# koide3/small_gicp

Hardware: AMD Instinct MI355X
Metric: GICP iterations/sec (1M<->1M pts) (higher is better)
Workload: dtype f32; 1 GPU; C3: GICP, per-point covariances k=20, 1000000 target <-> 1000000 source points, max_corr_dist 1.0 m; parallelism=single GPU

## Files before the change

### include/small_gicp_amd_debug.h

```cpp
#ifndef SMALL_GICP_AMD_DEBUG_H
#define SMALL_GICP_AMD_DEBUG_H

#include "small_gicp_amd.h"

#ifdef __cplusplus
extern "C" {
#endif

int sga_problem_set_search_stats(sga_context* ctx, sga_problem* pb, int enabled);
int sga_problem_get_search_stats(sga_context* ctx, const sga_problem* pb, int* leaves_per_point);
int sga_problem_get_sorted_points(sga_context* ctx, const sga_problem* pb, float* xyzw);
int sga_problem_get_last_plan(const sga_problem* pb, int out[8]);
int sga_problem_get_grid_stats(const sga_problem* pb, uint64_t out[6]);
void sga_set_grid_mode(int mode, long long min_points);
void sga_set_knn_wave_max(long long max_points);
int sga_index_spacing(const sga_index* index, double* spacing);
int sga_debug_kd_tree(sga_context* ctx, const sga_index* index, int* depth, float* nodes, float* xyzw);
int sga_debug_index_bbox(const sga_index* index, float lo[3], float hi[3]);
int sga_debug_forest_launches(unsigned long long* launches);
int sga_debug_voxelgrid_plan(const sga_cloud* cloud, double leaf, int out[9]);
int sga_debug_voxelgrid_batch_plan(const sga_cloud* const* clouds, size_t count, double leaf, int out[6]);
int sga_debug_voxelgrid_batch_launches(unsigned long long* launches);
int sga_debug_set_voxelgrid_epoch(sga_context* ctx, unsigned epoch);
int sga_debug_timer_start(sga_context* ctx);
int sga_debug_timer_stop(sga_context* ctx, double* ms);
#define SGA_FRAME_CHECK_DOUBLES 32
void sga_debug_shard_frame_pack(const double origin[3], double out[SGA_FRAME_CHECK_DOUBLES]);
// ... 11 lines not shown
```

### small_gicp_amd/_lib.py

```python
import ctypes as C
import os
import sys

_HERE = os.path.dirname(os.path.abspath(__file__))
LIB_PATH = os.environ.get("SGA_LIB_PATH") or os.path.join(_HERE, "lib", "libsmall_gicp_amd.so")

SGA_OK = 0
ICP, PLANE_ICP, GICP = 0, 1, 2
FLAT_NORMALS, FLAT_COVS = 1, 2
ROBUST_NONE, ROBUST_HUBER, ROBUST_CAUCHY = 0, 1, 2
LEVENBERG_MARQUARDT, GAUSS_NEWTON = 0, 1
MATH_FP32, MATH_FP64 = 0, 1
ACCUM_DOUBLES = 30


class SgaError(RuntimeError):
    pass


class FactorParams(C.Structure):
    _fields_ = [("factor_kind", C.c_int), ("robust_kind", C.c_int), ("robust_c", C.c_double), ("max_dist_sq", C.c_double), ("math_mode", C.c_int)]


class RegistrationSettingC(C.Structure):
# ... 112 lines not shown
    ("sga_linearize_per_point", C.c_int, [_vp, _vp, C.POINTER(FactorParams), _dp, _dp, C.POINTER(C.c_ubyte)]),
    ("sga_problem_get_factors", C.c_int, [_vp, _vp, C.POINTER(C.c_int64), _fp]),
    ("sga_context_set_stream_ordered", C.c_int, [_vp, C.c_int]),
    ("sga_context_set_profiling", C.c_int, [_vp, C.c_int]),
    ("sga_context_get_kernel_ms", C.c_int, [_vp, _dp, C.POINTER(C.c_uint64), _dp, C.POINTER(C.c_uint64)]),
    ("sga_context_get_comm_ms", C.c_int, [_vp, _dp, C.POINTER(C.c_uint64)]),
    ("sga_context_get_search_ms", C.c_int, [_vp, _dp, C.POINTER(C.c_uint64)]),
    ("sga_context_get_pass_ms", C.c_int, [_vp, _dp, C.POINTER(C.c_uint64), _dp, C.POINTER(C.c_uint64), _dp]),
    ("sga_set_warm_limit", None, [C.c_double]),
    ("sga_set_error_model", None, [C.c_int]),
    ("sga_problem_set_search_stats", C.c_int, [C.c_void_p, C.c_void_p, C.c_int]),
    ("sga_problem_get_search_stats", C.c_int, [C.c_void_p, C.c_void_p, C.c_void_p]),
    ("sga_problem_get_sorted_points", C.c_int, [C.c_void_p, C.c_void_p, C.c_void_p]),
    ("sga_problem_get_grid_stats", C.c_int, [C.c_void_p, C.POINTER(C.c_uint64)]),
    ("sga_problem_get_last_plan", C.c_int, [C.c_void_p, C.POINTER(C.c_int)]),
    ("sga_set_grid_mode", None, [C.c_int, C.c_longlong]),
    ("sga_host_alloc", C.c_int, [C.c_size_t, C.POINTER(C.c_void_p)]),
    ("sga_host_free", C.c_int, [C.c_void_p]),
    ("sga_index_spacing", C.c_int, [C.c_void_p, C.POINTER(C.c_double)]),
    ("sga_set_knn_wave_max", None, [C.c_longlong]),
    ("sga_debug_kd_tree", C.c_int, [C.c_void_p, C.c_void_p, C.POINTER(C.c_int), C.c_void_p, C.c_void_p]),
    ("sga_debug_voxelgrid_plan", C.c_int, [C.c_void_p, C.c_double, C.POINTER(C.c_int)]),
    ("sga_debug_set_voxelgrid_epoch", C.c_int, [C.c_void_p, C.c_uint]),
    ("sga_debug_timer_start", C.c_int, [C.c_void_p]),
    ("sga_debug_timer_stop", C.c_int, [C.c_void_p, C.POINTER(C.c_double)]),
    ("sga_debug_shard_frame_pack", None, [C.POINTER(C.c_double), C.POINTER(C.c_double)]),
    ("sga_debug_shard_frame_agree", C.c_int, [C.POINTER(C.c_double)]),
    ("sga_debug_reduce_rows", C.c_int, [C.c_void_p, C.c_void_p, C.c_int, C.c_int, C.c_void_p]),
    ("sga_debug_reduce_stamps", C.c_int, [C.c_void_p]),
    ("sga_debug_kd_trips", C.c_int, [C.c_void_p]),
# ... 60 lines not shown
```

### small_gicp_amd/api.py

```python
import ctypes as C

import numpy as np

from . import _lib
from ._lib import GICP, ICP, PLANE_ICP, FactorParams, RegistrationSettingC, ResultC, check, load

_FACTOR_BY_NAME = {"ICP": ICP, "PLANE_ICP": PLANE_ICP, "GICP": GICP, "VGICP": GICP}


def _fp(a):
    return None if a is None else a.ctypes.data_as(C.POINTER(C.c_float))


def _dp(a):
    return None if a is None else a.ctypes.data_as(C.POINTER(C.c_double))


def _T16(T):
    T = np.eye(4) if T is None else np.asarray(T, dtype=np.float64).reshape(4, 4)
    return np.ascontiguousarray(T.T).reshape(16)


class Context:

# ... 740 lines not shown
    def factors(self):
        n = self.source.size()
        ti = np.empty(n, np.int64)
        m6 = np.empty((n, 6), np.float32)
        check(load().sga_problem_get_factors(self.ctx.h, self.h, ti.ctypes.data_as(C.POINTER(C.c_int64)), _fp(m6)))
        return ti, m6

    ROUTES = ("factors", "grid", "certify", "fused_lane", "fused_queue", "queue", "lane")

    def last_plan(self):
        out = (C.c_int * 8)()
        check(load().sga_problem_get_last_plan(self.h, out))
        v = list(out)
        return {"route": self.ROUTES[v[0]], "warm": bool(v[1]), "grid": bool(v[2]), "pts": v[3], "tail": bool(v[4]), "chunk_tiles": v[5], "reduce_rows": v[6], "reduce_groups": v[7]}

    def align(self, setting, init_T=None):
        res = ResultC()
        t16 = _T16(init_T)
        check(load().sga_align_problem(self.ctx.h, self.h, _dp(t16), C.byref(setting), C.byref(res)))
        return RegistrationResult(res)

    def search_stats(self, enable=None):
        if enable is not None:
            check(load().sga_problem_set_search_stats(self.ctx.h, self.h, 1 if enable else 0))
            return None
        out = np.zeros(len(self.source), dtype=np.int32)
        check(load().sga_problem_get_search_stats(self.ctx.h, self.h, out.ctypes.data_as(C.c_void_p)))
        return out

    def sorted_points(self):
# ... 387 lines not shown
```

### small_gicp_amd/csrc/common.hpp

```cpp
#pragma once
#include <hip/hip_runtime.h>

#include <atomic>
#include <cstdarg>
#include <cstdint>
#include <cstdio>
#include <cstdlib>
#include <cstring>
#include <string>
#include <vector>

#include "../../include/small_gicp_amd.h"
#include "../../include/small_gicp_amd_debug.h"

namespace sga {

void set_error(const char* fmt, ...);
int fail(int code, const char* fmt, ...);

#define SGA_HIP(expr)                                                                                             \
  do {                                                                                                            \
    hipError_t _e = (expr);                                                                                       \
    if (_e != hipSuccess) return ::sga::fail(SGA_ERR_HIP, "%s:%d %s -> %s", __FILE__, __LINE__, #expr, hipGetErrorString(_e)); \
  } while (0)
// ... 218 lines not shown
  double src_origin[3] = {0, 0, 0};
  bool frame_checked = false;
  bool has_normals = false, has_covs = false;
  sga::DevBuf<float4> pts;
  sga::DevBuf<sga::Cov8> cov;
  const float4* pts_view = nullptr;
  const sga::Cov8* cov_view = nullptr;
  const float4* src_pts() const { return pts_view ? pts_view : pts.p; }
  const sga::Cov8* src_cov() const { return cov_view ? cov_view : cov.p; }
  sga::DevBuf<int> corr;
  sga::DevBuf<int> hint;
  sga::DevBuf<int> hint2;
  sga::DevBuf<float> rex;
  sga::DevBuf<int> dbg_leaves;
  sga::DevBuf<uint32_t> walked;
  bool state_fresh = false;
  double T_prev[16] = {0};
  bool prev_valid = false;
  int prev_math = 0;
  int lin_factor = -1;
  double lin_T[16] = {0};
  bool maha_valid = false;
  int last_math = 0;
  float bbox_lo[3] = {0, 0, 0}, bbox_hi[3] = {0, 0, 0};
  uint64_t cold_passes = 0, warm_passes = 0;
  uint64_t grid_passes = 0;
  sga::DevBuf<uint32_t> grid_stats;
  bool grid_stats_pending = false;
  uint64_t grid_open_total = 0, grid_ring_total = 0;
  double grid_open_frac = 0.0;
  sga::DevBuf<uint32_t> tile_cost, tile_order;
// ... 15 lines not shown
```

### small_gicp_amd/csrc/linearize.hip

```cpp
#include <algorithm>
#include <type_traits>

#include "batch.hpp"
#include "common.hpp"
#include "device_math.hpp"
#include "uniform.hpp"
#include "cell_grid.hpp"
#include "kd_search.hpp"
#include "projective.hpp"
#include "voxel_hash.hpp"
#include "notes.hpp"
#include "pass_layout.hpp"
#include "search_stage.hpp"
#include "factor_stage.hpp"
#include "reduce_rows.hpp"

void sga_profile_collect_pending(sga_context* ctx);

namespace sga {

int comm_allreduce_sum(sga_context* ctx, double* d_buf, size_t count);
template <typename Real>
int grid_search_pass(sga_context* ctx, const sga_index* idx, const float4* src_pts, int n, const Rigid<Real>& T, float reach2, int* nn, int* nn2, float* rex, uint32_t* stats);
int grid_rings_for(const sga_index* idx, double reach);
// ... 54 lines not shown
  uint32_t node = 1;
  int depth = 0, sp = 0;
  KdState s = kd_state(p.bound2, 0.f);

  for (;;) {
    while (tile < tile_end && q_count <= kQueueCap - 64) {
      const int i = tile * 64 + lane;
      bool need = i < p.n;
      float fx = 0.f, fy = 0.f, fz = 0.f, slack = 0.f;
      int seed = -1, cand2 = -1;
      if (need) {
        const float4 ps = p.src_pts[i];
        Real x, y, z;
        transform_point<Real>(p.T, ps.x, ps.y, ps.z, x, y, z);
        fx = static_cast<float>(x), fy = static_cast<float>(y), fz = static_cast<float>(z);
        seed = p.nn[i];
        cand2 = p.nn2[i];
        if constexpr (CHECK) {
          Real ox, oy, oz;
          transform_point<Real>(p.T_prev, ps.x, ps.y, ps.z, ox, oy, oz);
          const float moved = sqrtf(kd_dist2(static_cast<float>(ox), static_cast<float>(oy), static_cast<float>(oz), fx, fy, fz));
          float d1 = INFINITY, d2 = INFINITY;
          if (seed >= 0) {
            const float4 c = p.kd.pts[seed];
            d1 = kd_dist2(c.x, c.y, c.z, fx, fy, fz);
          }
          if (cand2 >= 0) {
            const float4 c = p.kd.pts[cand2];
            d2 = kd_dist2(c.x, c.y, c.z, fx, fy, fz);
          }
          const bool swap = cand2 >= 0 && (d2 < d1 || (d2 == d1 && cand2 < seed));
          const int best = swap ? cand2 : seed;
// ... 479 lines not shown
    acc += wave_sum_f64(static_cast<double>(e));
  }
  if (lane == 0) sh_e[wave] = acc;
  __syncthreads();
  if (threadIdx.x == 0) {
    double s = 0.0;
    for (int w = 0; w < kTile / 64; w++) s += sh_e[w];
    if (p.tail.enabled)
      __hip_atomic_store(&p.partials[blockIdx.x], s, __ATOMIC_RELAXED, __HIP_MEMORY_SCOPE_AGENT);
    else
      p.partials[blockIdx.x] = s;
  }
  if (p.tail.enabled) fused_tail(p.tail, p.partials, gridDim.x, 1, 1);
}

__global__ __launch_bounds__(1024) void tile_order_kernel(const uint32_t* __restrict__ cost, uint32_t* __restrict__ order, int num_tiles) {
  __shared__ uint32_t hist[64], start[64];
  const int per_xcd = num_tiles >> 3;
  const int x = blockIdx.x, first = x * per_xcd;
  if (threadIdx.x < 64) hist[threadIdx.x] = 0u;
  __syncthreads();
  for (int k = threadIdx.x; k < per_xcd; k += blockDim.x) atomicAdd(&hist[63u - min(63u, cost[first + k] >> 8)], 1u);
  __syncthreads();
  if (threadIdx.x == 0) {
    uint32_t acc = 0u;
    for (int b = 0; b < 64; b++) {
      start[b] = acc;
      acc += hist[b];
    }
  }
  __syncthreads();
  for (int k = threadIdx.x; k < per_xcd; k += blockDim.x) {
    const uint32_t pos = atomicAdd(&start[63u - min(63u, cost[first + k] >> 8)], 1u);
    order[first + pos] = static_cast<uint32_t>(first + k);
  }
  if (x == 0)
    for (int t = 8 * per_xcd + threadIdx.x; t < num_tiles; t += blockDim.x) order[t] = static_cast<uint32_t>(t);
}

template <typename T>
static T env_or(const char* name, T d) {
  const char* s = getenv(name);
  return s == nullptr ? d : std::is_floating_point_v<T> ? static_cast<T>(atof(s)) : static_cast<T>(atoll(s));
}

constexpr int kLinPts = 4;
constexpr int kLinPtsMin = 750000;
constexpr int kLinPtsMinF64 = 131072;

static double g_warm_delta = env_or("SGA_WARM_DELTA", 0.1);

static int g_search_queue = env_or("SGA_SEARCH_QUEUE", 2);
constexpr double kQueueDelta = 0.02;
static int g_chunk_tiles_cold = env_or("SGA_CHUNK_COLD", 4);
// ... 222 lines not shown

  const int math = sizeof(Real) == 4 ? SGA_MATH_FP32 : SGA_MATH_FP64;
  const double displacement = (!voxel && p.n > 0 && pb->prev_valid && pb->prev_math == math) ? max_displacement(T, pb->T_prev, pb->bbox_lo, pb->bbox_hi) : INFINITY;
  const double unit = voxel ? 1.0 : routing_unit(idx);
  NNParams<Real> q{};
  q.src_pts = pb->src_pts();
  q.n = p.n;
  q.kd = p.kd;
  q.T = p.T;
  q.within2 = p.bound2;
  q.slack_min = static_cast<float>(kSlackMin * unit), q.slack_max = static_cast<float>(kSlackMax * unit);
  q.cert_pad = std::max(g_cert_pad, 0.f);
  q.bound2 = p.bound2 * (1.f + kSearchMargin) * (1.f + kSearchMargin);
  q.nn = pb->hint.p, q.nn2 = pb->hint2.p, q.rex = pb->rex.p, q.walked = pb->walked.p;
  q.fast = g_fast_scan;
  q.leaves = pb->dbg_leaves.n >= pb->n ? pb->dbg_leaves.p : nullptr;

  const PassPlan plan = plan_pass<Real>(ctx, pb, q, displacement, unit, host_rejector);
  p.num_tiles = factor_tiles(p.n, plan.pts);
  const int blocks = grid_blocks(p.num_tiles);
  p.tail = FusedTail{plan.tail ? 1 : 0, ctx->d_ticket.p, d_out30, out_n, host, seq};
  q.check = plan.warm ? 1 : 0;
  if (plan.warm) q.T_prev = rigid_from_colmajor<Real>(pb->T_prev);
  if (plan.grid) {
    q.grid_walk = g_grid_walk;
    q.grid = make_grid_view(idx);
  }
  q.chunk_tiles = plan.chunk_tiles;

  const bool timed = ctx->profiling && (ctx->lin_seq++ % ctx->profile_period) == 0;
  if (timed) {
    sga_profile_collect_pending(ctx);
    (void)hipEventRecord(ctx->ev0, ctx->stream);
    ctx->pending_warm = plan.warm;
  }
  int rows = p.n > 0 ? blocks : 0;
  const bool first_pass = !pb->prev_valid;
  if (!voxel) pb->prev_valid = false;
  pb->state_fresh = false;
  if (plan.route != Route::kFactors) {
    if (q.leaves != nullptr) SGA_HIP(hipMemsetAsync(q.leaves, 0, pb->n * sizeof(int), ctx->stream));
    if (plan.grid && (first_pass || (plan.route != Route::kGrid && !plan.warm))) pb->grid_open_frac = 0.0;
    pb->order_tiles = 0;
    const size_t words = static_cast<size_t>(p.kd.depth);
    const dim3 sgrid((p.n + kSearchBlock - 1) / kSearchBlock), sblock(kSearchBlock);
    switch (plan.route) {
      case Route::kGrid:
        if (pb->grid_stats.n < 4) {
          SGA_TRY(pb->grid_stats.alloc(4));
          SGA_HIP(hipMemsetAsync(pb->grid_stats.p, 0, 4 * sizeof(uint32_t), ctx->stream));
        }
        SGA_TRY(grid_search_pass<Real>(ctx, idx, pb->src_pts(), p.n, p.T, q.bound2, pb->hint.p, pb->hint2.p, pb->rex.p, pb->grid_stats.p));
        pb->grid_passes++;
        break;
// ... 79 lines not shown
    }
  }
  if (p.n > 0 && !plan.fused()) {
    with_factor(fp->factor_kind, [&](auto f) {
      constexpr int F = decltype(f)::value;
      if (flat)
        launch_linearize<Real, F, 2>(ctx->stream, p, blocks, plan.pts);
      else if (proj) {
        hipLaunchKernelGGL((projective_linearize_kernel<Real, F, 1>), dim3(blocks), dim3(kTile), 0, ctx->stream, p, make_proj_view(idx));
      } else if (voxel) {
        if constexpr (F != SGA_PLANE_ICP) launch_linearize<Real, F, 1>(ctx->stream, p, blocks, plan.pts);
      } else
        launch_linearize<Real, F, 0>(ctx->stream, p, blocks, plan.pts);
    });
  }
  if (!plan.tail) launch_reduce(ctx, pb->partials.p, rows, ncols, kRow, pb->partials.p + partial_rows(pb->n) * kRow, d_out30, out_n, host, seq, true, plan.route == Route::kGrid ? pb->grid_stats.p : nullptr);
  pb->grid_stats_pending = plan.route == Route::kGrid && !plan.tail && out_n > kStatsCol + 1;
  {
    const int lp[8] = {static_cast<int>(plan.route), plan.warm, plan.grid, plan.pts, plan.tail, plan.chunk_tiles, plan.tail ? 0 : rows, plan.tail ? 0 : reduce_groups(rows)};
    std::copy(lp, lp + 8, pb->last_plan);
  }
  if (timed) {
    (void)hipEventRecord(ctx->ev1, ctx->stream);
    ctx->pending |= 1;
  }
  if (plan.order_record) {
    hipLaunchKernelGGL(tile_order_kernel, dim3(8), dim3(1024), 0, ctx->stream, pb->tile_cost.p, pb->tile_order.p, rows);
    pb->order_tiles = static_cast<unsigned>(rows);
    pb->order_stream = ctx->stream;
  }
  SGA_HIP(hipGetLastError());
  pb->last_math = math;
  pb->lin_factor = fp->factor_kind;
  memcpy(pb->lin_T, T, sizeof(pb->lin_T));
  pb->maha_valid = p.store_maha != 0;
  if (!voxel) {
    memcpy(pb->T_prev, T, sizeof(pb->T_prev));
    pb->prev_valid = true;
    pb->prev_math = math;
    if (plan.warm)
      pb->warm_passes++;
    else
// ... 331 lines not shown
    d.pair = k;
    prefix[a] = blocks;
    blocks += (d.ntiles + 7) / 8 * 8;
    pairs[a] = d;
  }
  prefix[order.size()] = blocks;
  const int nactive = static_cast<int>(order.size());
  const unsigned long long seq = ++bt->seq;
  SGA_HIP(hipMemcpyAsync(bt->d_round.p, bt->h_round, batch_round_bytes(count), hipMemcpyHostToDevice, ctx->stream));
  const int* d_prefix = reinterpret_cast<const int*>(bt->d_round.p);
  const BatchPair* d_pairs = reinterpret_cast<const BatchPair*>(bt->d_round.p + batch_pairs_offset(count));
  for (int k : order) {
    sga_problem* pb = bt->problems[k];
    pb->prev_valid = false;
    pb->model_valid = false;
    pb->state_fresh = false;
    pb->order_tiles = 0;
    if (bt->tiles[k] == 0 && pb->n > 0) SGA_HIP(hipMemsetAsync(pb->corr.p, 0xff, pb->n * sizeof(int), ctx->stream));
  }
  if (blocks > 0) {
    const size_t lds = static_cast<size_t>(std::max(bt->max_depth, 3)) * 64 * sizeof(uint32_t);
    with_factor(fp->factor_kind, [&](auto f) { hipLaunchKernelGGL((batch_search_linearize_kernel<decltype(f)::value>), dim3(blocks), dim3(64), lds, ctx->stream, d_prefix, d_pairs, nactive); });
  }
  hipLaunchKernelGGL(batch_reduce_rows_kernel, dim3(nactive), dim3(kReduceSlices * kCols), 0, ctx->stream, d_pairs, bt->ticket.p, bt->h_out_dev, bt->h_out_dev + count * kRow, seq);
  SGA_HIP(hipGetLastError());
  int rc = wait_result(ctx, seq, bt->h_out + count * kRow);
  if (rc != SGA_OK) {
    (void)hipMemsetAsync(bt->ticket.p, 0, sizeof(unsigned), ctx->stream);
    return rc;
  }
  for (size_t a = 0; a < order.size(); a++) {
// ... 84 lines not shown
  if (enabled) return pb->dbg_leaves.alloc(pb->n);
  pb->dbg_leaves.release();
  return SGA_OK;
}
int sga_problem_get_sorted_points(sga_context* ctx, const sga_problem* pb, float* xyzw) {
  if (!ctx || !pb || !xyzw) return fail(SGA_ERR_INVALID, "null argument");
  if (pb->n == 0) return SGA_OK;
  SGA_ENTER(ctx);
  SGA_HIP(hipMemcpyAsync(xyzw, pb->src_pts(), pb->n * sizeof(float4), hipMemcpyDeviceToHost, ctx->stream));
  SGA_HIP(hipStreamSynchronize(ctx->stream));
  return SGA_OK;
}
int sga_problem_get_last_plan(const sga_problem* pb, int out[8]) {
  if (!pb || !out) return fail(SGA_ERR_INVALID, "null argument");
  std::copy(pb->last_plan, pb->last_plan + 8, out);
  return SGA_OK;
}
int sga_problem_get_search_stats(sga_context* ctx, const sga_problem* pb, int* leaves_per_point) {
  if (!ctx || !pb || !leaves_per_point) return fail(SGA_ERR_INVALID, "null argument");
  if (pb->dbg_leaves.n < pb->n) return fail(SGA_ERR_INVALID, "search statistics are not enabled");
  SGA_ENTER(ctx);
  SGA_HIP(hipMemcpyAsync(leaves_per_point, pb->dbg_leaves.p, pb->n * sizeof(int), hipMemcpyDeviceToHost, ctx->stream));
  SGA_HIP(hipStreamSynchronize(ctx->stream));
  return SGA_OK;
}

int sga_debug_reduce_rows(sga_context* ctx, const double* rows, int nrows, int derive, double* out) {
  if (!ctx || !out || nrows < 0 || (nrows > 0 && !rows)) return fail(SGA_ERR_INVALID, "null argument or negative row count");
  SGA_ENTER(ctx);
  const size_t stage_off = sga::partial_rows(static_cast<size_t>(nrows) * 64) * sga::kRow;
// ... 44 lines not shown
#define SGA_PRELOAD_FACTOR(F)                                        \
  SGA_PRELOAD(search_linearize_kernel<float, F, false>);            \
  SGA_PRELOAD(search_linearize_kernel<float, F, true>);             \
  SGA_PRELOAD(nn_search_queue_kernel<float, true, F>);              \
  SGA_PRELOAD(certify_linearize_kernel<float, F, 1>);               \
  SGA_PRELOAD(linearize_kernel<float, F, 0, kLinPts>);              \
  SGA_PRELOAD(linearize_kernel<float, F, 0, 1>);                   \
  SGA_PRELOAD(batch_search_linearize_kernel<F>)
  SGA_PRELOAD_FACTOR(SGA_GICP);
  SGA_PRELOAD_FACTOR(SGA_PLANE_ICP);
  SGA_PRELOAD_FACTOR(SGA_ICP);
  SGA_PRELOAD(linearize_kernel<float, SGA_GICP, 1, kLinPts>);
  SGA_PRELOAD(linearize_kernel<float, SGA_GICP, 1, 1>);
  SGA_PRELOAD(reduce_rows_kernel);
  SGA_PRELOAD(batch_reduce_rows_kernel);
  SGA_PRELOAD(tile_order_kernel);
  SGA_PRELOAD(publish_kernel);
  SGA_PRELOAD(error_kernel<float, SGA_GICP>);
#undef SGA_PRELOAD_FACTOR
#undef SGA_PRELOAD
  (void)hipGetLastError();
}
}

extern "C" {

void sga_set_grid_mode(int mode, long long min_points) {
  if (mode >= 0) sga::g_grid_mode = mode;
  if (min_points >= 0) sga::g_grid_min_points = min_points;
}

// ... 8 lines not shown
```

### small_gicp_amd/csrc/multi.hip

```cpp
#include <memory>
#include <vector>

#include "common.hpp"

namespace sga {
int linearize_enqueue(sga_context* ctx, sga_problem* pb, const sga_factor_params* fp, const double T[16], unsigned long long* seq_out, int* count_out);
int linearize_collect(sga_context* ctx, sga_problem* pb, const double T[16], unsigned long long seq, int count);
int error_enqueue(sga_context* ctx, sga_problem* pb, const sga_factor_params* fp, const double T[16], unsigned long long* seq_out);
int error_collect(sga_context* ctx, unsigned long long seq, double* e);
double error_model_value(const double* acc96, const double T_lin[16], const double T[16]);
bool error_model_enabled();
const double* problem_pose(const sga_problem* pb, const double T[16], double Td[16]);
void problem_system_to_caller(const sga_problem* pb, double H[36], double b[6]);
int cloud_create_f32_about(sga_context* ctx, const float* xyz, const float* normals, const float* cov6, size_t n, const double origin[3], sga_cloud** out);
void host_bbox_f32(const float* xyz, size_t n, double lo[3], double hi[3]);
void host_bbox_f64(const double* xyzw, size_t n, double lo[3], double hi[3]);
}

using namespace sga;

struct sga_multi {
  struct Shard {
    int device = 0;
    sga_context* ctx = nullptr;
// ... 294 lines not shown
  return SGA_OK;
}

int sga_multi_get_factors(sga_multi* m, int64_t* target_index, float* mahalanobis6) {
  if (!m) return fail(SGA_ERR_INVALID, "null argument");
  if (!m->has_source) return fail(SGA_ERR_INVALID, "sga_multi_get_factors without clouds");
  for (auto& s : m->shards) {
    if (s.count == 0) continue;
    SGA_TRY(sga_problem_get_factors(s.ctx, s.problem, target_index ? target_index + s.first : nullptr, mahalanobis6 ? mahalanobis6 + 6 * s.first : nullptr));
  }
  return SGA_OK;
}

int sga_multi_reset_search_state(sga_multi* m) {
  if (!m) return fail(SGA_ERR_INVALID, "null argument");
  for (auto& s : m->shards) {
    if (!s.problem) continue;
    SGA_HIP(hipSetDevice(s.device));
    Entered in(s.ctx);
    sga_problem* pb = s.problem;
    if (pb->n > 0 && pb->hint.n >= pb->n) SGA_HIP(hipMemsetAsync(pb->hint.p, 0xff, pb->n * sizeof(int), s.ctx->stream));
    if (pb->n > 0 && pb->hint2.n >= pb->n) SGA_HIP(hipMemsetAsync(pb->hint2.p, 0xff, pb->n * sizeof(int), s.ctx->stream));
    pb->prev_valid = false;
  }
  m->model_valid = false;
  return SGA_OK;
}

int sga_multi_align(sga_multi* m, const double init_T[16], const sga_registration_setting* setting, sga_result* out) {
  if (!m || !setting || !out) return fail(SGA_ERR_INVALID, "null argument");
  if (!m->has_source) return fail(SGA_ERR_INVALID, "sga_multi_align without clouds");
  static const double I16[16] = {1, 0, 0, 0, 0, 1, 0, 0, 0, 0, 1, 0, 0, 0, 0, 1};
  if (m->n_target <= 10) std::fprintf(stderr, "warning: target point cloud is too small. |target|=%zu\n", m->n_target);
  if (m->n_source <= 10) std::fprintf(stderr, "warning: source point cloud is too small. |source|=%zu\n", m->n_source);
  SGA_TRY(sga_multi_reset_search_state(m));
  MultiReduction r{m, &setting->factor};
  return sga_optimize(setting, init_T ? init_T : I16, multi_lin_cb, multi_err_cb, &r, out);
}

// ... 13 lines not shown
```

### small_gicp_amd/csrc/optimizer.hip

```cpp
#include <cmath>
#include <cstdio>

#include "batch.hpp"
#include "common.hpp"

namespace sga {

struct M4 {
  double a[16];
};

static M4 mul(const M4& A, const M4& B) {
  M4 C;
  for (int c = 0; c < 4; c++)
    for (int r = 0; r < 4; r++) {
      double s = 0;
      for (int k = 0; k < 4; k++) s += A.a[4 * k + r] * B.a[4 * c + k];
      C.a[4 * c + r] = s;
    }
  return C;
}

static M4 se3_exp(const double d[6]) {
  const double wx = d[0], wy = d[1], wz = d[2];
// ... 352 lines not shown
  const M4 m = se3_exp(twist);
  memcpy(T, m.a, sizeof(m.a));
}

int sga_optimize(const sga_registration_setting* setting, const double init_T[16], sga_linearize_fn linearize, sga_error_fn error, void* user, sga_result* out) {
  if (!setting || !init_T || !linearize || !out) return fail(SGA_ERR_INVALID, "null argument");
  if (setting->optimizer == SGA_LEVENBERG_MARQUARDT && !error) return fail(SGA_ERR_INVALID, "LM needs an error callback");
  return optimize_impl(*setting, init_T, linearize, error, user, out);
}

int sga_align_problem(sga_context* ctx, sga_problem* problem, const double init_T[16], const sga_registration_setting* setting, sga_result* out) {
  if (!ctx || !problem || !setting || !out) return fail(SGA_ERR_INVALID, "null argument");
  static const double I16[16] = {1, 0, 0, 0, 0, 1, 0, 0, 0, 0, 1, 0, 0, 0, 0, 1};
  if (problem->target->n <= 10) std::fprintf(stderr, "warning: target point cloud is too small. |target|=%zu\n", problem->target->n);
  if (problem->n <= 10) std::fprintf(stderr, "warning: source point cloud is too small. |source|=%zu\n", problem->n);
  if (!problem->state_fresh) {
    SGA_HIP(hipSetDevice(ctx->device));
    if (problem->n > 0) SGA_HIP(hipMemsetAsync(problem->hint.p, 0xff, problem->n * sizeof(int), ctx->stream));
    if (problem->n > 0 && problem->hint2.n >= problem->n) SGA_HIP(hipMemsetAsync(problem->hint2.p, 0xff, problem->n * sizeof(int), ctx->stream));
  }
  problem->prev_valid = false;
  GpuReduction g{ctx, problem, &setting->factor};
  return optimize_impl(*setting, init_T ? init_T : I16, gpu_linearize, gpu_error, &g, out);
}

int sga_optimize_batch(const sga_registration_setting* setting, size_t count, const double* init_T, sga_batch_linearize_fn linearize, sga_batch_error_fn error, void* user, sga_result* out) {
  if (!setting || !linearize) return fail(SGA_ERR_INVALID, "null argument");
  if (setting->optimizer == SGA_LEVENBERG_MARQUARDT && !error) return fail(SGA_ERR_INVALID, "LM needs an error callback");
  if (count == 0) return SGA_OK;
  if (!out) return fail(SGA_ERR_INVALID, "null argument");
  return optimize_batch_impl(*setting, count, init_T, linearize, error, user, out);
}

int sga_align_batch(sga_context* ctx, sga_batch* batch, const double* init_T, const sga_registration_setting* setting, sga_result* out) {
  if (!setting) return fail(SGA_ERR_INVALID, "null argument");
// ... 25 lines not shown
```

### small_gicp_amd/csrc/pass_layout.hpp

```cpp
#pragma once
#include "cell_grid.hpp"
#include "common.hpp"
#include "device_math.hpp"
#include "kd_search.hpp"
#include "voxel_hash.hpp"

namespace sga {

constexpr int kTile = 256;
constexpr int kRow = 96;
constexpr int kCols = 128;
constexpr int kModelOff = 32;
constexpr int kModelCols = 95;
constexpr int kStatsCol = 30;
constexpr int kSearchBlock = 64;
#ifndef SGA_MAX_BLOCKS
#define SGA_MAX_BLOCKS 2048
#endif
constexpr int kMaxBlocks = SGA_MAX_BLOCKS;
constexpr int kReduceGroups = 64;
constexpr int kReduceSlices = 8;


constexpr int kFuseMaxBlocks = 32;
// ... 52 lines not shown
  float cert_pad;
  int* __restrict__ nn;
  int* __restrict__ nn2;
  float* __restrict__ rex;
  int check;
  Rigid<Real> T_prev;
  uint32_t* __restrict__ walked;
  const uint32_t* __restrict__ tile_order;
  uint32_t* __restrict__ tile_cost;
  int* __restrict__ leaves;
  double inv_leaf;
  int chunk_tiles;
  int fast;
  GridView grid;
  int grid_walk;
};

template <typename Real>
struct ErrParams {
  const float4* __restrict__ src_pts;
  int n;
  int num_tiles;
  const float4* __restrict__ tgt_pts;
  const float4* __restrict__ tgt_nrm;
  const int* __restrict__ corr;
  const Real* __restrict__ maha;
  Rigid<Real> T;
  int robust_kind;
  Real robust_c;
  double* __restrict__ partials;
// ... 14 lines not shown
```

### small_gicp_amd/csrc/problem.hip

```cpp
#include "common.hpp"

#include <cmath>
#include <memory>
#include <rocprim/rocprim.hpp>
#include "device_math.hpp"
#include "kd_search.hpp"
#include "sort_util.hpp"
#include "voxel_hash.hpp"

namespace sga {

int ensure_temp(sga_context* ctx, size_t bytes);
size_t problem_partials_doubles(size_t n);
int problem_ensure_maha(sga_context* ctx, sga_problem* pb);
int cloud_bbox(sga_context* ctx, const float4* pts, size_t n, float lo[3], float hi[3]);
int projective_source_keys(sga_context* ctx, const sga_index* idx, const float4* pts, size_t n, const double T_dev[16], unsigned long long* keys, uint32_t* vals);
int projective_index_knn(sga_context* ctx, const sga_index* index, const float* queries, const double* queries64, size_t m, int k, double max_sq_dist, int64_t* idx, float* sq_dist, double* sq_dist64);

__device__ __forceinline__ unsigned long long spread3(unsigned long long v) {
  v &= 0x1fffffull;
  v = (v | (v << 32)) & 0x1f00000000ffffull;
  v = (v | (v << 16)) & 0x1f0000ff0000ffull;
  v = (v | (v << 8)) & 0x100f00f00f00f00full;
  v = (v | (v << 4)) & 0x10c30c30c30c30c3ull;
// ... 215 lines not shown
  SGA_TRY(pb->partials.alloc(problem_partials_doubles(n)));
  SGA_TRY(pb->walked.alloc(n / 64 + 1));
  if (n > 0 && own_arrays) {
    SGA_TRY(pb->pts.alloc(n));
    if (has_covs) SGA_TRY(pb->cov.alloc(n));
  }
  if (n > 0) {
    SGA_TRY(pb->corr.alloc(n));
    SGA_TRY(pb->hint.alloc(n));
    SGA_TRY(pb->hint2.alloc(n));
    SGA_TRY(pb->rex.alloc(n));
    SGA_TRY(pb->maha.alloc(n * 6));
  }
  hipLaunchKernelGGL(problem_state_init_kernel, dim3((n + 255) / 256 + 1), dim3(256), 0, ctx->stream, pb->corr.p, pb->hint.p, pb->hint2.p, pb->walked.p, n);
  SGA_HIP(hipGetLastError());
  pb->state_fresh = true;
  return SGA_OK;
}

int sga_problem_create_from_index(sga_context* ctx, const sga_index* target, const sga_index* source, const double init_T[16], sga_problem** out) {
  if (!ctx || !target || !source || !out) return fail(SGA_ERR_INVALID, "null argument");
  if (target->device != ctx->device || source->device != ctx->device) return fail(SGA_ERR_INVALID, "target/source live on another device");
  if (source->kind == SGA_INDEX_PROJECTIVE) return fail(SGA_ERR_UNSUPPORTED, "a projective search cannot serve as the source index: pass its cloud");
  if (source->kind != SGA_INDEX_KDTREE) return fail(SGA_ERR_INVALID, "the source index must be a kd-tree");
  (void)init_T;
  *out = nullptr;
  SGA_ENTER(ctx);
  SGA_TRY(wait_ready(ctx, target->ready));
  SGA_TRY(wait_ready(ctx, source->ready));
  std::unique_ptr<sga_problem> pb(new sga_problem);
  pb->device = ctx->device;
// ... 220 lines not shown
```

### small_gicp_amd/csrc/reduce_rows.hpp

```cpp
#pragma once
#include <algorithm>

#include "pass_layout.hpp"
#include "uniform.hpp"

namespace sga {

__host__ __device__ inline double derived_entry(int col, const double* m) {
  auto S = [](int j, int k) { return static_cast<int>((0x542431210ull >> (4 * (3 * j + k))) & 15ull); };
  auto A = [&](int a, int j, int k) { return m[kModelOff + 9 + 6 * a + S(j, k)]; };
  auto B = [&](int a, int b, int j, int k) { return m[kModelOff + 27 + 6 * S(a, b) + S(j, k)]; };
  auto G = [&](int a, int j) { return m[kModelOff + 3 * a + j]; };
  auto PK = [&](int l, int i, int k) { const int i1 = (i + 1) % 3, i2 = (i + 2) % 3; return B(l, i1, i2, k) - B(l, i2, i1, k); };
  if (col >= 21) {
    const int i = col - 21, i1 = (i + 1) % 3, i2 = (i + 2) % 3;
    return G(i2, i1) - G(i1, i2);
  }
  const int i = col < 6 ? 0 : (col < 11 ? 1 : 2);
  const int j = col - (6 * i - i * (i - 1) / 2) + i;
  if (j >= 3) {
    const int k = j - 3, i1 = (i + 1) % 3, i2 = (i + 2) % 3;
    return A(i1, i2, k) - A(i2, i1, k);
  }
  const int j1 = (j + 1) % 3, j2 = (j + 2) % 3;
// ... 36 lines not shown
  if (f.host != nullptr) {
    __threadfence_system();
    __syncthreads();
    if (threadIdx.x == 0) __hip_atomic_store(reinterpret_cast<unsigned long long*>(f.host + kSeqWord), f.seq, __ATOMIC_RELEASE, __HIP_MEMORY_SCOPE_SYSTEM);
  }
}

#ifdef SGA_REDUCE_STAMPS
static __device__ unsigned long long g_reduce_stamps[24];
#define SGA_STAMP(k)                                                                         \
  do {                                                                                       \
    if (threadIdx.x == 0) {                                                                  \
      const unsigned long long stamp_now = wall_clock64();                                   \
      stamp_local[k] = stamp_now;                                                            \
      if (blockIdx.x == 0) g_reduce_stamps[k] = stamp_now;                                   \
      if (blockIdx.x == gridDim.x - 1) g_reduce_stamps[8 + (k)] = stamp_now;                 \
    }                                                                                        \
  } while (0)
#else
#define SGA_STAMP(k) ((void)0)
#endif

__global__ __launch_bounds__(kReduceSlices * kCols) void reduce_rows_kernel(
  const double* __restrict__ partials, int nrows, int ncols, int row_stride, double* __restrict__ stage, unsigned* __restrict__ ticket, double* __restrict__ out, int out_n, double* __restrict__ host,
  unsigned long long seq, int derive, const uint32_t* __restrict__ stats) {
  __shared__ double sh[kReduceSlices][kCols];
  __shared__ unsigned sh_ticket;
  const int c = threadIdx.x & (kCols - 1), s = threadIdx.x / kCols;
  const int G = gridDim.x;
#ifdef SGA_REDUCE_STAMPS
  unsigned long long stamp_local[6] = {0, 0, 0, 0, 0, 0};
#endif
  SGA_STAMP(0);
  double a0 = 0.0, a1 = 0.0, a2 = 0.0, a3 = 0.0;
  if (c < ncols) {
    const int step = G * kReduceSlices;
    int r = blockIdx.x + G * s;
    for (; r + 3 * step < nrows; r += 4 * step) {
      const double v0 = partials[static_cast<size_t>(r) * row_stride + c], v1 = partials[static_cast<size_t>(r + step) * row_stride + c];
      const double v2 = partials[static_cast<size_t>(r + 2 * step) * row_stride + c], v3 = partials[static_cast<size_t>(r + 3 * step) * row_stride + c];
      a0 += v0, a1 += v1, a2 += v2, a3 += v3;
    }
    for (; r < nrows; r += step) a0 += partials[static_cast<size_t>(r) * row_stride + c];
  }
// ... 42 lines not shown
      out[cc] = r;
      if (host != nullptr) host[cc] = r;
    }
  }
  if (G > 1 && threadIdx.x == 0) __hip_atomic_store(ticket, 0u, __ATOMIC_RELAXED, __HIP_MEMORY_SCOPE_AGENT);
  if (host != nullptr) {
    SGA_STAMP(4);
    if (threadIdx.x < kCols) __threadfence_system();
    __syncthreads();
    SGA_STAMP(5);
    if (threadIdx.x == 0) __hip_atomic_store(reinterpret_cast<unsigned long long*>(host + kSeqWord), seq, __ATOMIC_RELEASE, __HIP_MEMORY_SCOPE_SYSTEM);
  }
#ifdef SGA_REDUCE_STAMPS
  if (threadIdx.x == 0) {
    for (int k = 0; k < 6; k++) g_reduce_stamps[16 + k] = stamp_local[k];
    g_reduce_stamps[22] = blockIdx.x, g_reduce_stamps[23] = gridDim.x;
  }
#endif
}

__global__ __launch_bounds__(kReduceSlices * kCols) void batch_reduce_rows_kernel(const BatchPair* __restrict__ pairs, unsigned* __restrict__ ticket, double* __restrict__ host, double* __restrict__ seq_word, unsigned long long seq) {
  __shared__ double sh[kReduceSlices][kCols];
  __shared__ unsigned sh_ticket;
  const BatchPair* d = uniform_const(pairs + blockIdx.x);
  const double* __restrict__ partials = d->p.partials;
  const int nrows = d->ntiles, out_row = d->pair;
  const int c = threadIdx.x & (kCols - 1), s = threadIdx.x / kCols;
  double a0 = 0.0, a1 = 0.0, a2 = 0.0, a3 = 0.0;
  if (c < kModelCols) {
    constexpr int step = kReduceSlices;
    int r = s;
// ... 22 lines not shown
  __syncthreads();
  if (threadIdx.x == 0) sh_ticket = __hip_atomic_fetch_add(ticket, 1u, __ATOMIC_ACQ_REL, __HIP_MEMORY_SCOPE_AGENT);
  __syncthreads();
  if (sh_ticket != gridDim.x - 1) return;
  if (threadIdx.x == 0) {
    __hip_atomic_store(ticket, 0u, __ATOMIC_RELAXED, __HIP_MEMORY_SCOPE_AGENT);
    __threadfence_system();
    __hip_atomic_store(reinterpret_cast<unsigned long long*>(seq_word), seq, __ATOMIC_RELEASE, __HIP_MEMORY_SCOPE_SYSTEM);
  }
}

static size_t partial_rows(size_t n) { return std::max<size_t>(kMaxBlocks, (n + 63) / 64); }

static int reduce_groups(int nrows) { return nrows > 256 ? std::min(kReduceGroups, std::max(8, nrows / 128)) : 1; }

static void launch_reduce(sga_context* ctx, const double* partials, int nrows, int ncols, int row_stride, double* stage, double* out, int out_n, double* host, unsigned long long seq, bool derive = false, const uint32_t* stats = nullptr) {
  const int groups = reduce_groups(nrows);
  hipLaunchKernelGGL(reduce_rows_kernel, dim3(groups), dim3(kReduceSlices * kCols), 0, ctx->stream, partials, nrows, ncols, row_stride, stage, ctx->d_ticket.p, out, out_n, host, seq, derive ? 1 : 0, stats);
}

}
```

### small_gicp_amd/csrc/search_stage.hpp

```cpp
#pragma once
#include "pass_layout.hpp"

namespace sga {

__device__ __forceinline__ void tile_schedule(int num_tiles, int& first, int& stride, int& end, int nblocks = 0) {
  if (nblocks == 0) nblocks = gridDim.x;
  if (nblocks % 8 == 0 && num_tiles >= nblocks) {
    const int xcd = blockIdx.x & 7, slot = blockIdx.x >> 3, per_xcd_blocks = nblocks >> 3;
    const int t0 = static_cast<int>((static_cast<long long>(num_tiles) * xcd) >> 3);
    const int t1 = static_cast<int>((static_cast<long long>(num_tiles) * (xcd + 1)) >> 3);
    first = t0 + slot;
    stride = per_xcd_blocks;
    end = t1;
  } else {
    first = blockIdx.x;
    stride = nblocks;
    end = num_tiles;
  }
}

__device__ __forceinline__ float rex_from_r2(float r2) { return sqrtf(r2) * 0.9999995f; }

constexpr float kSearchMargin = 0.05f;

// ... 12 lines not shown
  if (!exact) {
    const KdBestFast f = kd_nearest_fast<BLOCK>(p.kd, fx, fy, fz, p.bound2, seed, kd_stack, tid, slack);
    nb = f.best;
    exact = f.ambiguous;
  }
  if (exact) nb = kd_nearest<BLOCK>(p.kd, fx, fy, fz, p.bound2, seed, kd_stack, tid, slack);
  p.nn[i] = nb.idx;
  p.nn2[i] = nb.idx2;
  p.rex[i] = rex_from_r2(nb.r2);
  if (p.leaves != nullptr) p.leaves[i] = nb.leaves;
  return nb.idx;
}

template <typename Real, int BLOCK, bool CHECK>
__device__ __forceinline__ int search_lane(const NNParams<Real>& p, int tile, int i, const float4& ps, float fx, float fy, float fz, uint32_t* __restrict__ kd_stack) {
  int seed = p.nn[i];
  float slack = 0.f;
  if constexpr (CHECK) {
    Real ox, oy, oz;
    transform_point<Real>(p.T_prev, ps.x, ps.y, ps.z, ox, oy, oz);
    const float moved = sqrtf(kd_dist2(static_cast<float>(ox), static_cast<float>(oy), static_cast<float>(oz), fx, fy, fz));
    const int cand2 = p.nn2[i];
    float d1 = INFINITY, d2 = INFINITY;
    if (seed >= 0) {
      const float4 c = p.kd.pts[seed];
      d1 = kd_dist2(c.x, c.y, c.z, fx, fy, fz);
    }
    if (cand2 >= 0) {
      const float4 c = p.kd.pts[cand2];
      d2 = kd_dist2(c.x, c.y, c.z, fx, fy, fz);
    }
// ... 42 lines not shown
```

Measured before the change: 9158 iterations/s.

## Fold tile-order sort into reduce launch and drop per-align hint memsets

Moves the per-XCD tile cost histogram sort out of its own kernel and into extra blocks appended to the reduce_rows launch, removing one kernel launch per pass. Also removes the hipMemsetAsync resets of hint/hint2 at align start and in multi-shard reset; instead, a new seedless flag makes the first (non-certified) pass ignore stale seeds. This saves memset launches and bandwidth, but relies on seedless handling being correct wherever stale hints could otherwise be read. A debug accessor for tile cost/order is added.

Result: no change. 9208 iterations/s, median of 4 (+0.5%).

```diff
diff --git a/include/small_gicp_amd_debug.h b/include/small_gicp_amd_debug.h
--- a/include/small_gicp_amd_debug.h
+++ b/include/small_gicp_amd_debug.h
@@ -11,6 +11,7 @@
 int sga_problem_get_search_stats(sga_context* ctx, const sga_problem* pb, int* leaves_per_point);
 int sga_problem_get_sorted_points(sga_context* ctx, const sga_problem* pb, float* xyzw);
 int sga_problem_get_last_plan(const sga_problem* pb, int out[8]);
+int sga_debug_problem_tile_order(sga_context* ctx, const sga_problem* pb, int* tiles, uint32_t* cost, uint32_t* order);
 int sga_problem_get_grid_stats(const sga_problem* pb, uint64_t out[6]);
 void sga_set_grid_mode(int mode, long long min_points);
 void sga_set_knn_wave_max(long long max_points);
diff --git a/small_gicp_amd/_lib.py b/small_gicp_amd/_lib.py
--- a/small_gicp_amd/_lib.py
+++ b/small_gicp_amd/_lib.py
@@ -150,6 +150,7 @@
     ("sga_problem_get_sorted_points", C.c_int, [C.c_void_p, C.c_void_p, C.c_void_p]),
     ("sga_problem_get_grid_stats", C.c_int, [C.c_void_p, C.POINTER(C.c_uint64)]),
     ("sga_problem_get_last_plan", C.c_int, [C.c_void_p, C.POINTER(C.c_int)]),
+    ("sga_debug_problem_tile_order", C.c_int, [C.c_void_p, C.c_void_p, C.POINTER(C.c_int), C.c_void_p, C.c_void_p]),
     ("sga_set_grid_mode", None, [C.c_int, C.c_longlong]),
     ("sga_host_alloc", C.c_int, [C.c_size_t, C.POINTER(C.c_void_p)]),
     ("sga_host_free", C.c_int, [C.c_void_p]),
diff --git a/small_gicp_amd/api.py b/small_gicp_amd/api.py
--- a/small_gicp_amd/api.py
+++ b/small_gicp_amd/api.py
@@ -778,6 +778,14 @@
         v = list(out)
         return {"route": self.ROUTES[v[0]], "warm": bool(v[1]), "grid": bool(v[2]), "pts": v[3], "tail": bool(v[4]), "chunk_tiles": v[5], "reduce_rows": v[6], "reduce_groups": v[7]}
 
+    def tile_order(self):
+        tiles = C.c_int()
+        check(load().sga_debug_problem_tile_order(self.ctx.h, self.h, C.byref(tiles), None, None))
+        cost, order = np.zeros(tiles.value, np.uint32), np.zeros(tiles.value, np.uint32)
+        if tiles.value > 0:
+            check(load().sga_debug_problem_tile_order(self.ctx.h, self.h, C.byref(tiles), cost.ctypes.data_as(C.c_void_p), order.ctypes.data_as(C.c_void_p)))
+        return cost, order
+
     def align(self, setting, init_T=None):
         res = ResultC()
         t16 = _T16(init_T)
diff --git a/small_gicp_amd/csrc/common.hpp b/small_gicp_amd/csrc/common.hpp
--- a/small_gicp_amd/csrc/common.hpp
+++ b/small_gicp_amd/csrc/common.hpp
@@ -256,7 +256,6 @@
   sga::DevBuf<float> rex;
   sga::DevBuf<int> dbg_leaves;
   sga::DevBuf<uint32_t> walked;
-  bool state_fresh = false;
   double T_prev[16] = {0};
   bool prev_valid = false;
   int prev_math = 0;
diff --git a/small_gicp_amd/csrc/linearize.hip b/small_gicp_amd/csrc/linearize.hip
--- a/small_gicp_amd/csrc/linearize.hip
+++ b/small_gicp_amd/csrc/linearize.hip
@@ -92,8 +92,10 @@
         Real x, y, z;
         transform_point<Real>(p.T, ps.x, ps.y, ps.z, x, y, z);
         fx = static_cast<float>(x), fy = static_cast<float>(y), fz = static_cast<float>(z);
-        seed = p.nn[i];
-        cand2 = p.nn2[i];
+        if (CHECK || !p.seedless) {
+          seed = p.nn[i];
+          cand2 = p.nn2[i];
+        }
         if constexpr (CHECK) {
           Real ox, oy, oz;
           transform_point<Real>(p.T_prev, ps.x, ps.y, ps.z, ox, oy, oz);
@@ -603,30 +605,6 @@
   if (p.tail.enabled) fused_tail(p.tail, p.partials, gridDim.x, 1, 1);
 }
 
-__global__ __launch_bounds__(1024) void tile_order_kernel(const uint32_t* __restrict__ cost, uint32_t* __restrict__ order, int num_tiles) {
-  __shared__ uint32_t hist[64], start[64];
-  const int per_xcd = num_tiles >> 3;
-  const int x = blockIdx.x, first = x * per_xcd;
-  if (threadIdx.x < 64) hist[threadIdx.x] = 0u;
-  __syncthreads();
-  for (int k = threadIdx.x; k < per_xcd; k += blockDim.x) atomicAdd(&hist[63u - min(63u, cost[first + k] >> 8)], 1u);
-  __syncthreads();
-  if (threadIdx.x == 0) {
-    uint32_t acc = 0u;
-    for (int b = 0; b < 64; b++) {
-      start[b] = acc;
-      acc += hist[b];
-    }
-  }
-  __syncthreads();
-  for (int k = threadIdx.x; k < per_xcd; k += blockDim.x) {
-    const uint32_t pos = atomicAdd(&start[63u - min(63u, cost[first + k] >> 8)], 1u);
-    order[first + pos] = static_cast<uint32_t>(first + k);
-  }
-  if (x == 0)
-    for (int t = 8 * per_xcd + threadIdx.x; t < num_tiles; t += blockDim.x) order[t] = static_cast<uint32_t>(t);
-}
-
 template <typename T>
 static T env_or(const char* name, T d) {
   const char* s = getenv(name);
@@ -879,6 +857,7 @@
   q.bound2 = p.bound2 * (1.f + kSearchMargin) * (1.f + kSearchMargin);
   q.nn = pb->hint.p, q.nn2 = pb->hint2.p, q.rex = pb->rex.p, q.walked = pb->walked.p;
   q.fast = g_fast_scan;
+  q.seedless = pb->prev_valid ? 0 : 1;
   q.leaves = pb->dbg_leaves.n >= pb->n ? pb->dbg_leaves.p : nullptr;
 
   const PassPlan plan = plan_pass<Real>(ctx, pb, q, displacement, unit, host_rejector);
@@ -902,7 +881,6 @@
   int rows = p.n > 0 ? blocks : 0;
   const bool first_pass = !pb->prev_valid;
   if (!voxel) pb->prev_valid = false;
-  pb->state_fresh = false;
   if (plan.route != Route::kFactors) {
     if (q.leaves != nullptr) SGA_HIP(hipMemsetAsync(q.leaves, 0, pb->n * sizeof(int), ctx->stream));
     if (plan.grid && (first_pass || (plan.route != Route::kGrid && !plan.warm))) pb->grid_open_frac = 0.0;
@@ -1012,7 +990,9 @@
         launch_linearize<Real, F, 0>(ctx->stream, p, blocks, plan.pts);
     });
   }
-  if (!plan.tail) launch_reduce(ctx, pb->partials.p, rows, ncols, kRow, pb->partials.p + partial_rows(pb->n) * kRow, d_out30, out_n, host, seq, true, plan.route == Route::kGrid ? pb->grid_stats.p : nullptr);
+  if (!plan.tail)
+    launch_reduce(ctx, pb->partials.p, rows, ncols, kRow, pb->partials.p + partial_rows(pb->n) * kRow, d_out30, out_n, host, seq, true, plan.route == Route::kGrid ? pb->grid_stats.p : nullptr,
+                  plan.order_record ? pb->tile_cost.p : nullptr, plan.order_record ? pb->tile_order.p : nullptr);
   pb->grid_stats_pending = plan.route == Route::kGrid && !plan.tail && out_n > kStatsCol + 1;
   {
     const int lp[8] = {static_cast<int>(plan.route), plan.warm, plan.grid, plan.pts, plan.tail, plan.chunk_tiles, plan.tail ? 0 : rows, plan.tail ? 0 : reduce_groups(rows)};
@@ -1023,7 +1003,6 @@
     ctx->pending |= 1;
   }
   if (plan.order_record) {
-    hipLaunchKernelGGL(tile_order_kernel, dim3(8), dim3(1024), 0, ctx->stream, pb->tile_cost.p, pb->tile_order.p, rows);
     pb->order_tiles = static_cast<unsigned>(rows);
     pb->order_stream = ctx->stream;
   }
@@ -1385,7 +1364,6 @@
     sga_problem* pb = bt->problems[k];
     pb->prev_valid = false;
     pb->model_valid = false;
-    pb->state_fresh = false;
     pb->order_tiles = 0;
     if (bt->tiles[k] == 0 && pb->n > 0) SGA_HIP(hipMemsetAsync(pb->corr.p, 0xff, pb->n * sizeof(int), ctx->stream));
   }
@@ -1500,6 +1478,16 @@
 int sga_problem_get_last_plan(const sga_problem* pb, int out[8]) {
   if (!pb || !out) return fail(SGA_ERR_INVALID, "null argument");
   std::copy(pb->last_plan, pb->last_plan + 8, out);
+  return SGA_OK;
+}
+int sga_debug_problem_tile_order(sga_context* ctx, const sga_problem* pb, int* tiles, uint32_t* cost, uint32_t* order) {
+  if (!ctx || !pb || !tiles) return fail(SGA_ERR_INVALID, "null argument");
+  *tiles = static_cast<int>(pb->order_tiles);
+  if (pb->order_tiles == 0) return SGA_OK;
+  SGA_ENTER(ctx);
+  if (cost) SGA_HIP(hipMemcpyAsync(cost, pb->tile_cost.p, pb->order_tiles * sizeof(uint32_t), hipMemcpyDeviceToHost, ctx->stream));
+  if (order) SGA_HIP(hipMemcpyAsync(order, pb->tile_order.p, pb->order_tiles * sizeof(uint32_t), hipMemcpyDeviceToHost, ctx->stream));
+  SGA_HIP(hipStreamSynchronize(ctx->stream));
   return SGA_OK;
 }
 int sga_problem_get_search_stats(sga_context* ctx, const sga_problem* pb, int* leaves_per_point) {
@@ -1574,7 +1562,6 @@
   SGA_PRELOAD(linearize_kernel<float, SGA_GICP, 1, 1>);
   SGA_PRELOAD(reduce_rows_kernel);
   SGA_PRELOAD(batch_reduce_rows_kernel);
-  SGA_PRELOAD(tile_order_kernel);
   SGA_PRELOAD(publish_kernel);
   SGA_PRELOAD(error_kernel<float, SGA_GICP>);
 #undef SGA_PRELOAD_FACTOR
diff --git a/small_gicp_amd/csrc/multi.hip b/small_gicp_amd/csrc/multi.hip
--- a/small_gicp_amd/csrc/multi.hip
+++ b/small_gicp_amd/csrc/multi.hip
@@ -332,15 +332,8 @@
 
 int sga_multi_reset_search_state(sga_multi* m) {
   if (!m) return fail(SGA_ERR_INVALID, "null argument");
-  for (auto& s : m->shards) {
-    if (!s.problem) continue;
-    SGA_HIP(hipSetDevice(s.device));
-    Entered in(s.ctx);
-    sga_problem* pb = s.problem;
-    if (pb->n > 0 && pb->hint.n >= pb->n) SGA_HIP(hipMemsetAsync(pb->hint.p, 0xff, pb->n * sizeof(int), s.ctx->stream));
-    if (pb->n > 0 && pb->hint2.n >= pb->n) SGA_HIP(hipMemsetAsync(pb->hint2.p, 0xff, pb->n * sizeof(int), s.ctx->stream));
-    pb->prev_valid = false;
-  }
+  for (auto& s : m->shards)
+    if (s.problem) s.problem->prev_valid = false;
   m->model_valid = false;
   return SGA_OK;
 }
diff --git a/small_gicp_amd/csrc/optimizer.hip b/small_gicp_amd/csrc/optimizer.hip
--- a/small_gicp_amd/csrc/optimizer.hip
+++ b/small_gicp_amd/csrc/optimizer.hip
@@ -390,11 +390,6 @@
   static const double I16[16] = {1, 0, 0, 0, 0, 1, 0, 0, 0, 0, 1, 0, 0, 0, 0, 1};
   if (problem->target->n <= 10) std::fprintf(stderr, "warning: target point cloud is too small. |target|=%zu\n", problem->target->n);
   if (problem->n <= 10) std::fprintf(stderr, "warning: source point cloud is too small. |source|=%zu\n", problem->n);
-  if (!problem->state_fresh) {
-    SGA_HIP(hipSetDevice(ctx->device));
-    if (problem->n > 0) SGA_HIP(hipMemsetAsync(problem->hint.p, 0xff, problem->n * sizeof(int), ctx->stream));
-    if (problem->n > 0 && problem->hint2.n >= problem->n) SGA_HIP(hipMemsetAsync(problem->hint2.p, 0xff, problem->n * sizeof(int), ctx->stream));
-  }
   problem->prev_valid = false;
   GpuReduction g{ctx, problem, &setting->factor};
   return optimize_impl(*setting, init_T ? init_T : I16, gpu_linearize, gpu_error, &g, out);
diff --git a/small_gicp_amd/csrc/pass_layout.hpp b/small_gicp_amd/csrc/pass_layout.hpp
--- a/small_gicp_amd/csrc/pass_layout.hpp
+++ b/small_gicp_amd/csrc/pass_layout.hpp
@@ -90,6 +90,7 @@
   int fast;
   GridView grid;
   int grid_walk;
+  int seedless;
 };
 
 template <typename Real>
diff --git a/small_gicp_amd/csrc/problem.hip b/small_gicp_amd/csrc/problem.hip
--- a/small_gicp_amd/csrc/problem.hip
+++ b/small_gicp_amd/csrc/problem.hip
@@ -253,7 +253,6 @@
   }
   hipLaunchKernelGGL(problem_state_init_kernel, dim3((n + 255) / 256 + 1), dim3(256), 0, ctx->stream, pb->corr.p, pb->hint.p, pb->hint2.p, pb->walked.p, n);
   SGA_HIP(hipGetLastError());
-  pb->state_fresh = true;
   return SGA_OK;
 }
 
diff --git a/small_gicp_amd/csrc/reduce_rows.hpp b/small_gicp_amd/csrc/reduce_rows.hpp
--- a/small_gicp_amd/csrc/reduce_rows.hpp
+++ b/small_gicp_amd/csrc/reduce_rows.hpp
@@ -74,20 +74,48 @@
       const unsigned long long stamp_now = wall_clock64();                                   \
       stamp_local[k] = stamp_now;                                                            \
       if (blockIdx.x == 0) g_reduce_stamps[k] = stamp_now;                                   \
-      if (blockIdx.x == gridDim.x - 1) g_reduce_stamps[8 + (k)] = stamp_now;                 \
+      if (static_cast<int>(blockIdx.x) == G - 1) g_reduce_stamps[8 + (k)] = stamp_now;       \
     }                                                                                        \
   } while (0)
 #else
 #define SGA_STAMP(k) ((void)0)
 #endif
 
+constexpr int kTileOrderGroups = 8;
+__device__ __forceinline__ void tile_order_share(const uint32_t* __restrict__ cost, uint32_t* __restrict__ order, int num_tiles, int x) {
+  __shared__ uint32_t hist[64], start[64];
+  const int per_xcd = num_tiles >> 3;
+  const int first = x * per_xcd;
+  if (threadIdx.x < 64) hist[threadIdx.x] = 0u;
+  __syncthreads();
+  for (int k = threadIdx.x; k < per_xcd; k += blockDim.x) atomicAdd(&hist[63u - min(63u, cost[first + k] >> 8)], 1u);
+  __syncthreads();
+  if (threadIdx.x == 0) {
+    uint32_t acc = 0u;
+    for (int b = 0; b < 64; b++) {
+      start[b] = acc;
+      acc += hist[b];
+    }
+  }
+  __syncthreads();
+  for (int k = threadIdx.x; k < per_xcd; k += blockDim.x) {
+    const uint32_t pos = atomicAdd(&start[63u - min(63u, cost[first + k] >> 8)], 1u);
+    order[first + pos] = static_cast<uint32_t>(first + k);
+  }
+  if (x == 0)
+    for (int t = 8 * per_xcd + threadIdx.x; t < num_tiles; t += blockDim.x) order[t] = static_cast<uint32_t>(t);
+}
+
 __global__ __launch_bounds__(kReduceSlices * kCols) void reduce_rows_kernel(
   const double* __restrict__ partials, int nrows, int ncols, int row_stride, double* __restrict__ stage, unsigned* __restrict__ ticket, double* __restrict__ out, int out_n, double* __restrict__ host,
-  unsigned long long seq, int derive, const uint32_t* __restrict__ stats) {
+  unsigned long long seq, int derive, const uint32_t* __restrict__ stats, int G, const uint32_t* __restrict__ tile_cost, uint32_t* __restrict__ tile_order) {
   __shared__ double sh[kReduceSlices][kCols];
   __shared__ unsigned sh_ticket;
+  if (static_cast<int>(blockIdx.x) >= G) {
+    tile_order_share(tile_cost, tile_order, nrows, static_cast<int>(blockIdx.x) - G);
+    return;
+  }
   const int c = threadIdx.x & (kCols - 1), s = threadIdx.x / kCols;
-  const int G = gridDim.x;
 #ifdef SGA_REDUCE_STAMPS
   unsigned long long stamp_local[6] = {0, 0, 0, 0, 0, 0};
 #endif
@@ -160,7 +188,7 @@
 #ifdef SGA_REDUCE_STAMPS
   if (threadIdx.x == 0) {
     for (int k = 0; k < 6; k++) g_reduce_stamps[16 + k] = stamp_local[k];
-    g_reduce_stamps[22] = blockIdx.x, g_reduce_stamps[23] = gridDim.x;
+    g_reduce_stamps[22] = blockIdx.x, g_reduce_stamps[23] = G;
   }
 #endif
 }
@@ -213,9 +241,11 @@
 
 static int reduce_groups(int nrows) { return nrows > 256 ? std::min(kReduceGroups, std::max(8, nrows / 128)) : 1; }
 
-static void launch_reduce(sga_context* ctx, const double* partials, int nrows, int ncols, int row_stride, double* stage, double* out, int out_n, double* host, unsigned long long seq, bool derive = false, const uint32_t* stats = nullptr) {
+static void launch_reduce(sga_context* ctx, const double* partials, int nrows, int ncols, int row_stride, double* stage, double* out, int out_n, double* host, unsigned long long seq, bool derive = false, const uint32_t* stats = nullptr,
+                          const uint32_t* tile_cost = nullptr, uint32_t* tile_order = nullptr) {
   const int groups = reduce_groups(nrows);
-  hipLaunchKernelGGL(reduce_rows_kernel, dim3(groups), dim3(kReduceSlices * kCols), 0, ctx->stream, partials, nrows, ncols, row_stride, stage, ctx->d_ticket.p, out, out_n, host, seq, derive ? 1 : 0, stats);
-}
-
-}
+  hipLaunchKernelGGL(reduce_rows_kernel, dim3(groups + (tile_order != nullptr ? kTileOrderGroups : 0)), dim3(kReduceSlices * kCols), 0, ctx->stream, partials, nrows, ncols, row_stride, stage, ctx->d_ticket.p, out, out_n, host, seq,
+                     derive ? 1 : 0, stats, groups, tile_cost, tile_order);
+}
+
+}
diff --git a/small_gicp_amd/csrc/search_stage.hpp b/small_gicp_amd/csrc/search_stage.hpp
--- a/small_gicp_amd/csrc/search_stage.hpp
+++ b/small_gicp_amd/csrc/search_stage.hpp
@@ -50,7 +50,7 @@
 
 template <typename Real, int BLOCK, bool CHECK>
 __device__ __forceinline__ int search_lane(const NNParams<Real>& p, int tile, int i, const float4& ps, float fx, float fy, float fz, uint32_t* __restrict__ kd_stack) {
-  int seed = p.nn[i];
+  int seed = (!CHECK && p.seedless) ? -1 : p.nn[i];
   float slack = 0.f;
   if constexpr (CHECK) {
     Real ox, oy, oz;
```
